# quzefan/LuSh-NeRF

Measured on AMD Instinct MI355X. Metric: training rays/sec (fwd+bwd), N_samples=64+64, higher is better.
Workload: dtype f16 MFMA forward (one fp16 plane per operand, fp32 accumulate; render outputs within 3e-5 of the fp32 reference); backward fp16 MFMA (one plane, per-launch power-of-two loss scale), fp32 accumulate; 1 GPU; poster_lushnerf 1xMI355X N_rand=4096/GPU N_samples=64 N_importance=64 blur kernel (DSK/RBK) on, fwd+bwd+Adam, one RCCL all-reduce of the flat gradient (BASELINE config C2); rays_per_gpu=4096, marched_rays_per_gpu=20480, planes_fwd=fp16x1, parallelism=dp1

## Files before the change

lush_nerf_amd/csrc/lush_mlp_dev.h:

```cpp
#pragma once
#include "lush_common.h"
#include "lush_mlp.h"

namespace lush {

__device__ __forceinline__ void lds_barrier() { asm volatile("s_waitcnt lgkmcnt(0)\n\ts_barrier" ::: "memory"); }

__device__ __forceinline__ unsigned mask_relayout(unsigned own, unsigned other, int h) {
    const unsigned w0 = h ? other : own, w1 = h ? own : other;
    const int sh = 4 * h;
    return ((w0 >> sh) & 0xFu) | (((w1 >> sh) & 0xFu) << 4) | (((w0 >> (8 + sh)) & 0xFu) << 8) | (((w1 >> (8 + sh)) & 0xFu) << 12);
}
__device__ __forceinline__ long long mask_index(int tile, int n_ml, int ml, int nrb, int rb, int CB, int cb) {
    return ((((long long)tile * CB + cb) * n_ml + ml) * nrb + rb) * 16;
}

template <int NS, int DT>
__device__ __forceinline__ void pe_put(char* img, int plane_bytes, int row_bytes, int pt, int col, float v) {
    __bf16 p[NS];
    split_planes<NS, DT>(v, p);
#pragma unroll
    for (int s = 0; s < NS; ++s)
        *reinterpret_cast<__bf16*>(img + s * plane_bytes + swz(pt, col >> 3, row_bytes) + (col & 7) * 2) = p[s];
}

__device__ __forceinline__ void point_of(const float* __restrict__ rays, const float* __restrict__ z,
                                         int S, long long gpt, float (&x)[3], float (&d)[3]) {
    const long long ray = gpt / S;
    const float zz = z[gpt];
    const float* rr = rays + ray * 11;
#pragma unroll
    for (int i = 0; i < 3; ++i) {
        x[i] = __fadd_rn(rr[i], __fmul_rn(rr[3 + i], zz));
        d[i] = rr[8 + i];
    }
}

__device__ __forceinline__ void lush_sincos(float x, float* sn, float* cs) {
    const float j = __builtin_rintf(__fmul_rn(x, 0.6366197723675814f));
    float r = __fmaf_rn(-j, 1.5707963705062866f, x);
    r = __fmaf_rn(-j, -4.371139000186243e-08f, r);
    r = __fmaf_rn(-j, -1.7151245100059906e-15f, r);
    const float z = __fmul_rn(r, r);
    float ps = __fmaf_rn(z, 0.0000027183114939898219064f, -0.000198393348360966317347f);
    ps = __fmaf_rn(z, ps, 0.0083333293858894631756f);
    ps = __fmaf_rn(z, ps, -0.166666666416265235595f);
    const float s = __fmaf_rn(__fmul_rn(z, r), ps, r);
    float pc = __fmaf_rn(z, 0.0000243904487962774090654f, -0.00138867637746099294692f);
    pc = __fmaf_rn(z, pc, 0.0416666233237390631894f);
    pc = __fmaf_rn(z, pc, -0.499999997251031003120f);
    const float c = __fmaf_rn(z, pc, 1.0f);
    const int q = (int)j;
    const float a = (q & 1) ? c : s, b = (q & 1) ? s : c;
    *sn = (q & 2) ? -a : a;
    *cs = ((q + 1) & 2) ? -b : b;
}

__device__ __forceinline__ void rev_split(float x, float* hi, float* lo) {
    constexpr float C_HI = 0.15915494309189535f;
    constexpr float C_LO = (float)(0.15915494309189533576888 - (double)C_HI);
    *hi = x * C_HI;
    *lo = __builtin_fmaf(x, C_HI, -*hi) + x * C_LO;
}
__device__ __forceinline__ void sincos_rev(float hi, float lo, int k, float* sn, float* cs) {
    const float s = (float)(1 << k);
    const float r = __builtin_amdgcn_fractf(hi * s) + lo * s;
    *sn = __builtin_amdgcn_sinf(r);
    *cs = __builtin_amdgcn_cosf(r);
}

template <int NS, int MT, int NTHREADS, int DT>
__device__ __noinline__ void pe_tile(char* peimg, int plane_bytes, int row_bytes, const float* rays, const float* z,
                                        int S, int P, long long tile_pt0, int tid, const int* live = nullptr) {
    constexpr int PARTS = NTHREADS / MT;
    const int pt = tid % MT, part = tid / MT;
    const long long gpt = tile_pt0 + pt;
    float x[3] = {0.f, 0.f, 0.f}, d[3] = {0.f, 0.f, 0.f};
    if (gpt < P) point_of(rays, z, S, live ? (long long)live[gpt] : gpt, x, d);
    for (int u = part; u < L_X + L_D; u += PARTS) {
        const bool isd = u >= L_X;
        const int k = isd ? u - L_X : u;
        const int base = isd ? PE_X : 0;
        const float f = (float)(1 << k);
#pragma unroll
        for (int i = 0; i < 3; ++i) {
            const float v = isd ? d[i] : x[i];
            if (k == 0) pe_put<NS, DT>(peimg, plane_bytes, row_bytes, pt, base + i, v);
            float s, c;
            lush_sincos(v * f, &s, &c);
            pe_put<NS, DT>(peimg, plane_bytes, row_bytes, pt, base + 3 + 6 * k + i, s);
            pe_put<NS, DT>(peimg, plane_bytes, row_bytes, pt, base + 3 + 6 * k + 3 + i, c);
        }
    }
    if (part == PARTS - 1) {
        pe_put<NS, DT>(peimg, plane_bytes, row_bytes, pt, PE_X_VALID, 0.f);
#pragma unroll
        for (int c = PE_X + PE_D_VALID; c < PE_X + PE_D; ++c) pe_put<NS, DT>(peimg, plane_bytes, row_bytes, pt, c, 0.f);
    }
}

__device__ __forceinline__ void dma16(const void* gptr, unsigned lds_base ) {
    unsigned keep;
    asm volatile("s_mov_b32 %0, m0\n\ts_mov_b32 m0, %2\n\ts_nop 0\n\tglobal_load_lds_dwordx4 %1, off\n\ts_mov_b32 m0, %0"
                 : "=&s"(keep) : "v"(gptr), "s"(lds_base) : "memory");
}

__device__ __forceinline__ void dma16s(const void* sbase , unsigned voff, unsigned lds_base ) {
    unsigned keep;
    asm volatile("s_mov_b32 %0, m0\n\ts_mov_b32 m0, %3\n\ts_nop 0\n\tglobal_load_lds_dwordx4 %1, %2\n\ts_mov_b32 m0, %0"
                 : "=&s"(keep) : "v"(voff), "s"(sbase), "s"(lds_base) : "memory");
}

__device__ __forceinline__ void dma16s_stream(const void* sbase , unsigned voff, unsigned lds_base ) {
    unsigned keep;
    asm volatile("s_mov_b32 %0, m0\n\ts_mov_b32 m0, %3\n\ts_nop 0\n\tglobal_load_lds_dwordx4 %1, %2 nt\n\ts_mov_b32 m0, %0"
                 : "=&s"(keep) : "v"(voff), "s"(sbase), "s"(lds_base) : "memory");
}

__device__ __forceinline__ void dma16s_x2(const void* sbase, unsigned voff0, unsigned lds0, unsigned voff1, unsigned lds1) {
    unsigned keep;
    asm volatile("s_mov_b32 %0, m0\n\ts_mov_b32 m0, %3\n\ts_nop 0\n\tglobal_load_lds_dwordx4 %1, %2\n\t"
                 "s_mov_b32 m0, %5\n\ts_nop 0\n\tglobal_load_lds_dwordx4 %4, %2\n\ts_mov_b32 m0, %0"
                 : "=&s"(keep) : "v"(voff0), "s"(sbase), "s"(lds0), "v"(voff1), "s"(lds1) : "memory");
}

}
```

lush_nerf_amd/csrc/lush_mlp_wide.hip:

```cpp
#include "lush_mlp_wide.h"
#include "lush_host.h"

#include <cstdio>
#include <cstdlib>
#include <utility>

namespace lush {

constexpr int WD_PE_PITCH = PE_ROW * 2 + 16;
constexpr int WD_PE_PLANE = WD_MT * WD_PE_PITCH;
constexpr int WD_PE_LIVE = (PE_X + PE_D) * 2;
static_assert(WD_PE_LIVE + 4 <= WD_PE_PITCH, "a row has room for the point's grid index");
constexpr int WD_SB = 2;
enum { WB_NONE = 0, WB_REG = 1, WB_PEX = 2, WB_PED = 3 };
enum { WC_NONE = 0, WC_ACT = 1, WC_ALPHA = 2 };

constexpr int WD_WRAP = NetNerf::fwd4_len / 8;
static_assert(NetNerf::fwd4_len % 8 == 0, "the quarter-row stream is whole positions");
constexpr int WD_TR_JUMP = 4 + 7 * 16 + 4;
constexpr int WD_TR_ALPHA = WD_TR_JUMP + 16;
constexpr int WD_TR_WRAP = WD_TR_JUMP + 2;
static_assert(WD_TR_ALPHA + 2 + 10 + 1 == WD_WRAP && WD_TR_WRAP == 122, "trunk | feature | alpha | views | rgb");
static_assert(WD_S < WD_TR_JUMP, "the prologue's positions are plain trunk positions");

LUSH_CLOCK_DECL(lush_clock_wide_fwd)

struct WdRt {
    bool pre_on;
    unsigned clamp;
    char* mptr[2];
    unsigned lane2;
    const float* nextbias;
    char* tile;
    char* srows;
    unsigned soff[2];
    unsigned srow_off;
};

typedef __attribute__((ext_vector_type(2))) unsigned short u16x2;
struct WdConvTmp {
    unsigned o[4];
    unsigned m;
    unsigned word[4];
};

template <int NRQP, int KB0, bool MASK>
struct WdConv {
    static constexpr int NB = 2 * NRQP;
    static constexpr int UPT = MASK ? 8 : 4;
    static constexpr int UPB = 2 * UPT;
    static constexpr int NVU = NB * UPB;

    template <int K>
    static __device__ __forceinline__ void unit(f32x16 (&pend)[2][2], u32x4 (&xout)[2][16], WdConvTmp& t, unsigned clamp) {
        constexpr int b = K / UPB, r = K % UPB, tt = r / UPT, u = r % UPT;
        constexpr int c = b % 2, rbl = b / 2, kb = KB0 + 2 * rbl + tt;
        constexpr int kind = MASK ? ((u == 0 || u == 1 || u == 3 || u == 5) ? 0 : 1) : 0;
        constexpr int i = MASK ? (kind == 0 ? (u == 0 ? 0 : (u == 1 ? 1 : (u == 3 ? 2 : 3))) : (u == 2 ? 0 : (u == 4 ? 1 : (u == 6 ? 2 : 3)))) : u;
        if constexpr (kind == 0) {
            unsigned o;
            asm volatile("v_cvt_pk_f16_f32 %0, %1, %2\n\tv_pk_max_i16 %0, %0, %3"
                         : "=&v"(o) : "v"(pend[c][rbl][8 * tt + 2 * i]), "v"(pend[c][rbl][8 * tt + 2 * i + 1]), "s"(clamp));
            t.o[i] = o;
            if constexpr (i == 3) {
                const u32x4 v = {t.o[0], t.o[1], t.o[2], t.o[3]};
                xout[c][kb] = v;
            }
        } else {
            constexpr int sh = 8 * tt + 2 * i;
            unsigned z;
            if constexpr (tt == 0 && i == 0) {
                asm volatile("v_pk_sub_u16 %0, 1, %1 op_sel_hi:[0,1] clamp" : "=v"(t.m) : "v"(t.o[i]));
            } else if constexpr (tt == 1 && i == 3) {
                unsigned w;
                asm volatile("v_pk_sub_u16 %1, 1, %3 op_sel_hi:[0,1] clamp\n\tv_lshl_or_b32 %2, %1, %4, %2\n\tv_lshrrev_b32 %1, 15, %2\n\tv_or_b32 %1, %1, %2\n\tv_not_b32 %0, %1"
                             : "=v"(w), "=&v"(z), "+v"(t.m) : "v"(t.o[i]), "n"(sh));
                t.word[b] = w;
            } else {
                asm volatile("v_pk_sub_u16 %0, 1, %2 op_sel_hi:[0,1] clamp\n\tv_lshl_or_b32 %1, %0, %3, %1" : "=&v"(z), "+v"(t.m) : "v"(t.o[i]), "n"(sh));
            }
        }
    }
};


template <int NRQ, int NPOS, int BMAIN, int KB0, int PRE, int CK, int NRQP, int CKB0, bool MASK, int NRQN, int D, int PQ, bool STASH, int LD, bool TRUNK = false>
struct WdPass {
    static constexpr int KBPP = 8 / NRQ;
    static constexpr int NG = NPOS * 16;
    static constexpr int DG = D < NG ? D : NG;
    using CV = WdConv<NRQP, CKB0, MASK>;
    static constexpr int NBLK = CK == WC_ACT ? CV::NB : 0;
    static constexpr int IPB = CK == WC_ACT ? CV::UPB + 5 : 0;
    static constexpr int NIT = NBLK * IPB;
    static_assert(BMAIN == WB_REG || NPOS == 1, "a PE-image segment is one position");
    static_assert(!STASH || NPOS == 4, "the stash pipeline is laid out over the 16 positions of a layer");

    struct Regs {
        bf16x8 a1[4];
        u32x4 bpe[2][4];
        WdConvTmp ct;
        unsigned dma_dst, dma_off;
    };

    static constexpr int ST_JOBS = 8;
    static constexpr bool st_write(int g) { return STASH && g % 16 >= 12 && (4 * PQ + g / 16) < ST_JOBS; }
    static constexpr bool st_read(int g) { return STASH && g % 16 >= 12 && (4 * PQ + g / 16) >= 1 && (4 * PQ + g / 16) <= ST_JOBS; }
    static constexpr int st_store_job(int g) {
        const int P = 4 * PQ + g / 16, m = g % 16;
        const int J = m >= 14 ? P - 1 : (m < 2 ? P - 2 : -1);
        return (STASH && J >= 0 && J < ST_JOBS) ? J : -1;
    }
    static constexpr int st_store_row(int g) { return g % 16 >= 14 ? g % 16 - 14 : g % 16 + 2; }
    static constexpr bool st_store(int g) { return st_store_job(g) >= 0; }

    static constexpr int item_weight(int k) {
        const int r = k % (IPB > 0 ? IPB : 1), b = k / (IPB > 0 ? IPB : 1);
        if (r < CV::UPB) {
            if (!MASK) return 3;
            const int u = r % CV::UPT;
            return (u == 0 || u == 1 || u == 3 || u == 5) ? 3 : 2;
        }
        if (r == CV::UPB) return MASK ? 2 : 0;
        return (b / 2) < NRQN ? 1 : 0;
    }
    static constexpr int fixed_load(int g) {
        const int m = g % 16;
        int w = 0;
        if (m < 4) w += 1;
        if (m == 4 || m == 5) w += 3;
        if (m == 8) w += 10;
        if (m >= 9 && m <= 11) w += 1;
        if (st_write(g)) w += 1;
        if (st_read(g)) w += 1;
        if (st_store(g)) w += 2;
        return w;
    }
    struct Sched {
        int first[NG + 1];
        int cap;
    };
    static constexpr Sched make_sched() {
        Sched S{};
        for (int cap = 6; cap < 64; ++cap) {
            int k = 0;
            for (int g = 0; g < NG; ++g) {
                S.first[g] = k;
                int load = fixed_load(g);
                if (g < DG || g == NG - 1) {
                    while (k < NIT) {
                        const int w = item_weight(k);
                        if (w > 0 && load + w > cap && !(g == NG - 1)) break;
                        load += w;
                        ++k;
                    }
                }
            }
            S.first[NG] = k;
            S.cap = cap;
            int last = 0;
            for (int g = 0; g < NG; ++g)
                if (S.first[g + 1] > S.first[g]) last = g;
            if (k == NIT && (last < DG || NIT == 0)) return S;
        }
        return S;
    }
    static constexpr Sched SC = make_sched();

    template <int SRC, int NKB>
    static __device__ __forceinline__ void load_bpe(Regs& r, const char* peimg, int row0, int lane) {
        const int n = lane & 31, hh = lane >> 5;
        const char* p = peimg + (row0 + n) * WD_PE_PITCH + hh * 16;
#pragma unroll
        for (int c = 0; c < 2; ++c)
#pragma unroll
            for (int k = 0; k < NKB; ++k)
                r.bpe[c][k] = *reinterpret_cast<const u32x4*>(p + c * 32 * WD_PE_PITCH + ((SRC == WB_PED ? PE_X / 8 : 0) + 2 * k) * 16);
    }

    template <int SRC, int NRQ_, int I, int M>
    static __device__ __forceinline__ void mfma(f32x16 (&act)[2][2], const Regs& r, const WdCarry& cr, const u32x4 (&xin)[2][16]) {
        constexpr int u = M / 2, c = M % 2;
        constexpr int kbl = NRQ_ == 2 ? u / 2 : u, rbl = NRQ_ == 2 ? u % 2 : 0;
        const bf16x8 a = u < 4 ? cr.a0[u] : r.a1[u - 4];
        if constexpr (SRC == WB_REG) act[c][rbl] = mfma_f16(a, __builtin_bit_cast(bf16x8, xin[c][KB0 + I * (8 / NRQ_) + kbl]), act[c][rbl]);
        else act[c][rbl] = mfma_f16(a, __builtin_bit_cast(bf16x8, r.bpe[c][SRC == WB_PED ? kbl % 2 : kbl]), act[c][rbl]);
    }

    template <int M>
    static __device__ __forceinline__ void fixed(WdCtx& cx, Regs& r, WdCarry& cr, const char* rd, const char* rd_next) {
        if constexpr (M < 4) {
            r.a1[M] = *reinterpret_cast<const bf16x8*>(rd + (4 + M) * 1024 + cx.lane * 16);
        } else if constexpr (M == 4) {
            r.dma_dst = cx.dma_base + cx.slot_off;
            r.dma_off = cx.fetch_off;
        } else if constexpr (M == 5) {
            if constexpr (TRUNK) {
                const unsigned f = cx.fetch_off + WD_SLOT == (unsigned)WD_TR_JUMP * WD_SLOT ? (unsigned)WD_TR_ALPHA * WD_SLOT : cx.fetch_off + WD_SLOT;
                cx.fetch_off = f == (unsigned)(WD_TR_ALPHA + 2) * WD_SLOT ? 0u : f;
            } else {
                cx.fetch_off = cx.fetch_off + WD_SLOT == (unsigned)WD_WRAP * WD_SLOT ? 0u : cx.fetch_off + WD_SLOT;
            }
            cx.slot_off = cx.slot_off + WD_SLOT == (unsigned)WD_S * WD_SLOT ? 0u : cx.slot_off + WD_SLOT;
        } else if constexpr (M == 8) {
            wd_dma_pair(cx.gbase + r.dma_off, cx.gbase + r.dma_off + 4096u, cx.voff, r.dma_dst, r.dma_dst + 4096u);
            cr.a0[0] = *reinterpret_cast<const bf16x8*>(rd_next + cx.lane * 16);
        } else if constexpr (M >= 9 && M <= 11) {
            cr.a0[M - 8] = *reinterpret_cast<const bf16x8*>(rd_next + (M - 8) * 1024 + cx.lane * 16);
        }
    }

    template <int K>
    static __device__ __forceinline__ void item(f32x16 (&pend)[2][2], u32x4 (&xout)[2][16], Regs& r, const WdRt& rt, int lane) {
        constexpr int b = K / IPB, rr = K % IPB, c = b % 2, rbl = b / 2;
        if constexpr (rr < CV::UPB) {
            CV::template unit<b * CV::UPB + rr>(pend, xout, r.ct, rt.clamp);
        } else if constexpr (rr == CV::UPB) {
            if constexpr (MASK) *reinterpret_cast<unsigned short*>(rt.mptr[c] + rbl * 128 + rt.lane2) = (unsigned short)r.ct.word[b];
        } else if constexpr (rbl < NRQN) {
            constexpr int j = rr - CV::UPB;
            const f32x4 v = *reinterpret_cast<const f32x4*>(rt.nextbias + rbl * 32 + 8 * (lane >> 5) + (j == 1 ? 0 : j == 2 ? 4 : j == 3 ? 16 : 20));
#pragma unroll
            for (int e = 0; e < 4; ++e) pend[c][rbl][4 * (j - 1) + e] = v[e];
        }
    }

    template <int G>
    static __device__ __forceinline__ void pending(f32x16 (&pend)[2][2], u32x4 (&xout)[2][16], Regs& r, const WdRt& rt, int lane, float (&alpha)[2]) {
        if constexpr (CK == WC_ACT) {
            wd_unroll<SC.first[G], SC.first[G + 1]>([&](auto kc) __attribute__((always_inline)) { item<decltype(kc)::value>(pend, xout, r, rt, lane); });
        } else if constexpr (CK == WC_ALPHA) {
            if constexpr (G == 0) {
                alpha[0] = pend[0][0][0];
                alpha[1] = pend[1][0][0];
            }
            if constexpr (G == 1) {
                asm volatile("" ::"v"(pend[0][0]), "v"(pend[1][0]));
            }
            if constexpr (G >= 1 && G <= 8) {
                constexpr int q = G - 1, c = q % 2, rbl = (q / 2) % 2, jj = q / 4;
                if constexpr (rbl < NRQN) {
#pragma unroll
                    for (int j2 = 0; j2 < 2; ++j2) {
                        const int j = 1 + 2 * jj + j2;
                        const f32x4 v = *reinterpret_cast<const f32x4*>(rt.nextbias + rbl * 32 + 8 * (lane >> 5) + (j == 1 ? 0 : j == 2 ? 4 : j == 3 ? 16 : 20));
#pragma unroll
                        for (int e = 0; e < 4; ++e) pend[c][rbl][4 * (j - 1) + e] = v[e];
                    }
                }
            }
        }
    }

    template <int JOB, int I4>
    static __device__ __forceinline__ void stash_store(const WdCarry& cr, const WdRt& rt) {
        constexpr int c = JOB / 4, j = JOB % 4;
        __builtin_nontemporal_store(cr.sb[I4 % WD_SB], reinterpret_cast<u32x4*>(rt.srows + ((c * 32 + 8 * I4) * LD + j * 64) * 2 + rt.srow_off));
    }
    template <int G>
    static __device__ __forceinline__ void stash(const u32x4 (&xin)[2][16], WdCarry& cr, const WdRt& rt, int lane) {
        constexpr int P = 4 * PQ + G / 16, m = G % 16;
        if constexpr (st_store(G)) stash_store<st_store_job(G), st_store_row(G)>(cr, rt);
        if constexpr (st_write(G)) {
            constexpr int job = P, c = job / 4, j = job % 4, o = m - 12;
            const int n = lane & 31, hh = lane >> 5;
            *reinterpret_cast<u32x4*>(rt.tile + (job % 2) * 4096 + n * 128 + (((2 * o + hh) ^ (n & 7)) << 4)) = xin[c][4 * j + o];
        }
        if constexpr (st_read(G)) {
            constexpr int job = P - 1, i = m - 12;
            const int row = 8 * i + (lane >> 3);
            cr.sb[i % WD_SB] = *reinterpret_cast<const u32x4*>(rt.tile + (job % 2) * 4096 + row * 128 + (((lane & 7) ^ (row & 7)) << 4));
        }
    }

    static constexpr int stores_in(int g0, int g1) {
        int n = 0;
        for (int g = g0 < 0 ? 0 : g0; g < g1 && g < NG; ++g) {
            if (st_store(g)) ++n;
            if (CK == WC_ACT && MASK)
                for (int k = SC.first[g]; k < SC.first[g + 1]; ++k)
                    if (k % IPB == CV::UPB) ++n;
        }
        return n;
    }

    template <int SRC, int NRQ_, int I, bool MAIN>
    static __device__ __forceinline__ void position(WdCtx& cx, f32x16 (&act)[2][2], f32x16 (&pend)[2][2], const u32x4 (&xin)[2][16],
                                                    u32x4 (&xout)[2][16], Regs& r, WdCarry& cr, const char* peimg, int row0, const WdRt& rt,
                                                    float (&alpha)[2]) {
        if constexpr (SRC != WB_REG) load_bpe<SRC, (SRC == WB_PED ? 2 : 4)>(r, peimg, row0, cx.lane);
        const char* rd = cx.ring + cx.slot_off;
        __builtin_amdgcn_sched_barrier(0);
        wd_unroll<0, 8>([&](auto mc) __attribute__((always_inline)) {
            constexpr int M = decltype(mc)::value;
            mfma<SRC, NRQ_, I, M>(act, r, cr, xin);
            fixed<M>(cx, r, cr, rd, nullptr);
            if constexpr (MAIN) {
                stash<16 * I + M>(xin, cr, rt, cx.lane);
                pending<16 * I + M>(pend, xout, r, rt, cx.lane, alpha);
            }
            __builtin_amdgcn_sched_barrier(0);
        });
        constexpr int younger = 2 * (WD_S - 2) + (MAIN ? stores_in(16 * (I + 1 - WD_S) + 8, 16 * I + 8) : 0);
        wd_wait_vm<(younger < 63 ? younger : 63)>();
        lds_barrier();
        const char* rd_next = cx.ring + cx.slot_off;
        __builtin_amdgcn_sched_barrier(0);
        wd_unroll<8, 16>([&](auto mc) __attribute__((always_inline)) {
            constexpr int M = decltype(mc)::value;
            mfma<SRC, NRQ_, I, M>(act, r, cr, xin);
            fixed<M>(cx, r, cr, rd, rd_next);
            if constexpr (MAIN) {
                stash<16 * I + M>(xin, cr, rt, cx.lane);
                pending<16 * I + M>(pend, xout, r, rt, cx.lane, alpha);
            }
            __builtin_amdgcn_sched_barrier(0);
        });
    }

    static __device__ __forceinline__ void run(WdCtx& cx, f32x16 (&act)[2][2], f32x16 (&pend)[2][2], const u32x4 (&xin)[2][16],
                                               u32x4 (&xout)[2][16], WdCarry& cr, const char* peimg, int row0, const WdRt& rt, float (&alpha)[2]) {
        Regs r;
        if constexpr (PRE == WB_PEX) {
            if (rt.pre_on) position<WB_PEX, 2, 0, false>(cx, act, pend, xin, xout, r, cr, peimg, row0, rt, alpha);
        } else if constexpr (PRE == WB_PED) {
            position<WB_PED, 2, 0, false>(cx, act, pend, xin, xout, r, cr, peimg, row0, rt, alpha);
        }
        wd_unroll<0, NPOS>([&](auto ic) __attribute__((always_inline)) {
            position<BMAIN, NRQ, decltype(ic)::value, true>(cx, act, pend, xin, xout, r, cr, peimg, row0, rt, alpha);
        });

    }
};

__device__ __noinline__ void wd_pe_tile(char* peimg, const float* rays, const float* z, int S, int P, long long tile_pt0, int tid, float* xd,
                                        const int* live) {
    const long long gpt = tile_pt0 + tid;
    float x[3] = {0.f, 0.f, 0.f}, d[3] = {0.f, 0.f, 0.f};
    if (gpt < P) point_of(rays, z, S, live ? (long long)live[gpt] : gpt, x, d);
    if (xd != nullptr) {
        float4* o = reinterpret_cast<float4*>(xd + gpt * 8);
        o[0] = make_float4(x[0], x[1], x[2], 0.f);
        o[1] = make_float4(d[0], d[1], d[2], 0.f);
    }
    float v[PE_X + PE_D];
#pragma unroll
    for (int c = 0; c < PE_X + PE_D; ++c) v[c] = 0.f;
#pragma unroll
    for (int i = 0; i < 3; ++i) {
        v[i] = x[i];
        v[PE_X + i] = d[i];
        float hx, lx, hd, ld;
        rev_split(x[i], &hx, &lx);
        rev_split(d[i], &hd, &ld);
#pragma unroll
        for (int k = 0; k < L_X; ++k) sincos_rev(hx, lx, k, &v[3 + 6 * k + i], &v[3 + 6 * k + 3 + i]);
#pragma unroll
        for (int k = 0; k < L_D; ++k) sincos_rev(hd, ld, k, &v[PE_X + 3 + 6 * k + i], &v[PE_X + 3 + 6 * k + 3 + i]);
    }
    char* row = peimg + tid * WD_PE_PITCH;
    if (live) *reinterpret_cast<int*>(row + WD_PE_LIVE) = gpt < P ? live[gpt] : 0;
#pragma unroll
    for (int c = 0; c < (PE_X + PE_D) / 8; ++c) {
        u32x4 w;
#pragma unroll
        for (int j = 0; j < 4; ++j) {
            unsigned o[1];
            split_pair<1, DT_F16>(v[8 * c + 2 * j], v[8 * c + 2 * j + 1], o);
            w[j] = o[0];
        }
        *reinterpret_cast<u32x4*>(row + c * 16) = w;
    }
}

__device__ __forceinline__ void wd_bias(f32x16 (&acc)[2][2], const float* b, int h, int nrq) {
#pragma unroll
    for (int c = 0; c < 2; ++c)
#pragma unroll
        for (int rbl = 0; rbl < 2; ++rbl) {
            if (rbl < nrq) {
                const f32x4* p = reinterpret_cast<const f32x4*>(b + rbl * 32 + 8 * h);
                const f32x4 v0 = p[0], v1 = p[1], v2 = p[4], v3 = p[5];
#pragma unroll
                for (int e = 0; e < 4; ++e) {
                    acc[c][rbl][e] = v0[e];
                    acc[c][rbl][4 + e] = v1[e];
                    acc[c][rbl][8 + e] = v2[e];
                    acc[c][rbl][12 + e] = v3[e];
                }
            }
        }
}

template <class N, int SPK, bool TRUNK = false>
__global__ __launch_bounds__(WD_NT) void mlp_wide_fwd_kernel(const MlpFwdArgs A) {
    static_assert(N::HW == 256 && N::NL == 8 && N::HV == 128, "the wide kernel is built for the 8x256 net");
    static_assert(!TRUNK || SPK == 0, "the trunk-only pass over all points keeps no stash");
    static_assert(!TRUNK || N::SKIP < N::NL - 1,"layer 7 of the trunk-only pass is a plain layer");
    constexpr int HW = N::HW, HV = N::HV, NL = N::NL, NRB = N::NRB;
    constexpr int NBIAS = N::f32_w_rgb;
    constexpr bool MASK = SPK > 0;
    constexpr int ML_BYTES = NRB * 128;
    constexpr int CB_BYTES = N::n_mask_layers * ML_BYTES;
    LUSH_CLOCK_STAMP(lush_clock_wide_fwd, 0);
    extern __shared__ __attribute__((aligned(16))) char smem[];
    float* biasl = reinterpret_cast<float*>(smem);
    char* ring = smem + NBIAS * 4;
    char* stage = ring + WD_S * WD_SLOT;
    char* peimg = stage + 8 * 4096;

    const int tid = threadIdx.x, lane = tid & 63;
    const int w = __builtin_amdgcn_readfirstlane(tid >> 6);
    const int n = lane & 31, h = lane >> 5;
    const char* wbase = reinterpret_cast<const char*>(A.wpk);
    {
        const float* f32 = reinterpret_cast<const float*>(wbase + (long long)N::total_entries * 1024);
        for (int i = tid; i < NBIAS; i += WD_NT) biasl[i] = f32[i];
    }
    WdCtx cx;
    cx.ring = ring;
    cx.ring_lds = (unsigned)(size_t)(__attribute__((address_space(3))) char*)ring;
    cx.gbase = wbase + (long long)N::fwd4_base * 1024;
    cx.slot_off = 0;
    cx.fetch_off = (unsigned)(WD_S % WD_WRAP) * WD_SLOT;
    cx.dma_base = __builtin_amdgcn_readfirstlane(cx.ring_lds + (unsigned)w * 1024u);
    cx.w = w;
    cx.lane = lane;
    cx.voff = (unsigned)lane * 16u + (unsigned)w * 1024u;
#pragma unroll
    for (int j = 0; j < WD_S; ++j)
        wd_dma_pair(cx.gbase + (unsigned)j * WD_SLOT, cx.gbase + (unsigned)j * WD_SLOT + 4096u, cx.voff, cx.dma_base + (unsigned)j * WD_SLOT, cx.dma_base + (unsigned)j * WD_SLOT + 4096u);

    const int row0 = w * 64;
    WdRt rt;
    rt.tile = stage + w * 8192;
    rt.pre_on = false;
    rt.srows = nullptr;
#pragma unroll
    for (int c = 0; c < 2; ++c) rt.soff[c] = (unsigned)(((c * 32 + n) * HW + h * 8) * 2);
    rt.srow_off = (unsigned)(((lane >> 3) * HW + (lane & 7) * 8) * 2);
    rt.lane2 = (unsigned)lane * 2u;
    float alpha[2] = {0.f, 0.f};
    int P = A.P, n_tiles = A.n_tiles;
    if (A.live_cnt != nullptr) {
        P = __builtin_amdgcn_readfirstlane(*A.live_cnt);
        n_tiles = (P + WD_MT - 1) / WD_MT;
    }

    for (int tile = blockIdx.x; tile < n_tiles; tile += gridDim.x) {
        const long long pt0 = (long long)tile * WD_MT;
        const long long wpt = pt0 + row0;
        wd_pe_tile(peimg, A.rays, A.z, A.S, P, pt0, tid, (SPK > 0 && !A.pe_rows) ? A.xd : nullptr, A.live_idx);
        if (tile == (int)blockIdx.x) wd_wait_vm<2 * (WD_S - 1)>();
        else wd_wait_vm<2 * (WD_S - 1) + (SPK > 0 ? 17 : 1)>();
        lds_barrier();
        if (SPK > 0 && A.pe_rows) {
            for (int i = tid; i < WD_MT * 12; i += WD_NT) {
                const int c = i % 12, pt = i / 12;
                const uint4 v = *reinterpret_cast<const uint4*>(peimg + pt * WD_PE_PITCH + c * 16);
                *reinterpret_cast<uint4*>(A.pe + (pt0 + pt) * PE_ROW + c * 8) = v;
            }
        }
        {
            unsigned long long gb = (unsigned long long)cx.gbase;
            asm volatile("" : "+s"(gb));
            cx.gbase = (const char*)gb;
        }
        char* mbase[2];
#pragma unroll
        for (int c = 0; c < 2; ++c) mbase[c] = reinterpret_cast<char*>(A.mask) + (wpt / 32 + c) * CB_BYTES;
        char* mdummy = reinterpret_cast<char*>(A.mask_dummy);
        auto mset = [&](int ml, int rb, bool dummy) __attribute__((always_inline)) {
#pragma unroll
            for (int c = 0; c < 2; ++c) rt.mptr[c] = dummy ? mdummy + c * 256 : mbase[c] + ml * ML_BYTES + rb * 128;
        };

        f32x16 accA[2][2], accB[2][2];
        u32x4 B0[2][16], B1[2][16];
        WdCarry a0;
#pragma unroll
        for (int i = 0; i < 4; ++i) a0.a0[i] = *reinterpret_cast<const bf16x8*>(cx.ring + cx.slot_off + i * 1024 + lane * 16);
        const float* btr = biasl + N::f32_b_trunk;
        wd_bias(accA, btr, h, 2);
        wd_bias(accB, btr + 64, h, 2);

        rt.clamp = 0u;
        WdPass<2, 1, WB_PEX, 0, WB_NONE, WC_NONE, 2, 0, MASK, 2, 16, 0, false, HW, TRUNK>::run(cx, accA, accB, B0, B0, a0, peimg, row0, rt, alpha);
        mset(0, 0, false); rt.nextbias = btr + 128;
        WdPass<2, 1, WB_PEX, 0, WB_NONE, WC_ACT, 2, 0, MASK, 2, 16, 0, false, HW, TRUNK>::run(cx, accB, accA, B0, B0, a0, peimg, row0, rt, alpha);
        mset(0, 2, false); rt.nextbias = btr + 192;
        WdPass<2, 1, WB_PEX, 0, WB_NONE, WC_ACT, 2, 4, MASK, 2, 16, 0, false, HW, TRUNK>::run(cx, accA, accB, B0, B0, a0, peimg, row0, rt, alpha);
        mset(0, 4, false); rt.nextbias = btr + HW;
        WdPass<2, 1, WB_PEX, 0, WB_NONE, WC_ACT, 2, 8, MASK, 2, 16, 0, false, HW, TRUNK>::run(cx, accB, accA, B0, B0, a0, peimg, row0, rt, alpha);

        auto layer = [&](int l, u32x4 (&xin)[2][16], u32x4 (&xout)[2][16]) __attribute__((always_inline)) {
            const bool feat = l == NL;
            const float* bl = btr + l * HW;
            rt.pre_on = l == N::SKIP;
            rt.srows = reinterpret_cast<char*>(A.h0 + (long long)(l - 1) * A.h_stride + wpt * HW);
            rt.clamp = 0u; mset(l - 1, 6, false); rt.nextbias = bl + 64;
            WdPass<2, 4, WB_REG, 0, WB_PEX, WC_ACT, 2, 12, MASK, 2, 48, 0, (SPK > 0), HW, TRUNK>::run(cx, accA, accB, xin, xin, a0, peimg, row0, rt, alpha);
            rt.clamp = feat ? 0x80008000u : 0u;
            mset(l, 0, feat); rt.nextbias = bl + 128;
            WdPass<2, 4, WB_REG, 0, WB_PEX, WC_ACT, 2, 0, MASK, 2, 60, 1, (SPK > 0), HW, TRUNK>::run(cx, accB, accA, xin, xout, a0, peimg, row0, rt, alpha);
            mset(l, 2, feat); rt.nextbias = bl + 192;
            WdPass<2, 4, WB_REG, 0, WB_PEX, WC_ACT, 2, 4, MASK, 2, 60, 2, (SPK > 0), HW, TRUNK>::run(cx, accA, accB, xin, xout, a0, peimg, row0, rt, alpha);
            mset(l, 4, feat); rt.nextbias = (feat || (TRUNK && l == NL - 1)) ? biasl + N::f32_b_alpha : bl + HW;
            WdPass<2, 4, WB_REG, 0, WB_PEX, WC_ACT, 2, 8, MASK, 2, 60, 3, (SPK > 0), HW, TRUNK>::run(cx, accB, accA, xin, xout, a0, peimg, row0, rt, alpha);
        };
#pragma unroll 1
        for (int l2 = 0; l2 < (TRUNK ? NL / 2 - 1 : NL / 2); ++l2) {
            layer(1 + 2 * l2, B0, B1);
            layer(2 + 2 * l2, B1, B0);
        }
        if constexpr (TRUNK) {
            layer(NL - 1, B0, B1);
            {
                WdConvTmp ct;
                using CV = WdConv<2, 12, false>;
                wd_unroll<0, CV::NVU>([&](auto kc) __attribute__((always_inline)) { CV::template unit<decltype(kc)::value>(accB, B1, ct, 0u); });
            }
            rt.pre_on = false;
            WdPass<1, 2, WB_REG, 0, WB_NONE, WC_NONE, 2, 0, false, 2, 16, 0, false, HW, TRUNK>::run(cx, accA, accB, B1, B1, a0, peimg, row0, rt, alpha);
            if (h == 0) {
#pragma unroll
                for (int c = 0; c < 2; ++c) {
                    const long long gpt = wpt + c * 32 + n;
                    if (gpt < P) *reinterpret_cast<float4*>(A.raw + gpt * 4) = make_float4(0.f, 0.f, 0.f, accA[c][0][0]);
                }
            }
            continue;
        }
        rt.pre_on = false;
        rt.clamp = 0x80008000u; mset(0, 0, true); rt.nextbias = biasl + N::f32_b_views;
        WdPass<1, 2, WB_REG, 0, WB_NONE, WC_ACT, 2, 12, MASK, 2, 32, 0, false, HW, TRUNK>::run(cx, accA, accB, B1, B0, a0, peimg, row0, rt, alpha);
        rt.nextbias = biasl + N::f32_b_views + 64;
        WdPass<2, 4, WB_REG, 0, WB_PED, WC_ALPHA, 1, 0, MASK, 2, 60, 0, false, HW, TRUNK>::run(cx, accB, accA, B0, B0, a0, peimg, row0, rt, alpha);
        rt.clamp = 0u; mset(NL, 0, false); rt.nextbias = biasl + N::f32_b_rgb;
        WdPass<2, 4, WB_REG, 0, WB_PED, WC_ACT, 2, 0, MASK, 1, 60, 0, false, HW, TRUNK>::run(cx, accA, accB, B0, B1, a0, peimg, row0, rt, alpha);
        {
            WdConvTmp ct;
            using CV = WdConv<2, 4, MASK>;
            mset(NL, 2, false);
            wd_unroll<0, CV::NVU>([&](auto kc) __attribute__((always_inline)) { CV::template unit<decltype(kc)::value>(accA, B1, ct, 0u); });
            if constexpr (MASK) {
#pragma unroll
                for (int b = 0; b < 4; ++b) *reinterpret_cast<unsigned short*>(rt.mptr[b % 2] + (b / 2) * 128 + rt.lane2) = (unsigned short)ct.word[b];
            }
        }
        if constexpr (SPK > 0) {
            char* hvrows = reinterpret_cast<char*>(A.hv + wpt * HV);
#pragma unroll
            for (int c = 0; c < 2; ++c)
#pragma unroll
                for (int j = 0; j < N::KKV / 4; ++j) {
#pragma unroll
                    for (int kq = 0; kq < 4; ++kq)
                        *reinterpret_cast<u32x4*>(rt.tile + n * 128 + (((2 * kq + h) ^ (n & 7)) << 4)) = B1[c][4 * j + kq];
#pragma unroll
                    for (int i = 0; i < 4; ++i) {
                        const int row = 8 * i + (lane >> 3);
                        const u32x4 v = *reinterpret_cast<const u32x4*>(rt.tile + row * 128 + (((lane & 7) ^ (row & 7)) << 4));
                        __builtin_nontemporal_store(v, reinterpret_cast<u32x4*>(hvrows + ((c * 32 + 8 * i) * HV + j * 64) * 2 + (unsigned)(((lane >> 3) * HV + (lane & 7) * 8) * 2)));
                    }
                }
        }
        WdPass<1, 1, WB_REG, 0, WB_NONE, WC_NONE, 2, 0, MASK, 2, 16, 0, false, HW, TRUNK>::run(cx, accB, accA, B1, B1, a0, peimg, row0, rt, alpha);
        if (h == 0) {
#pragma unroll
            for (int c = 0; c < 2; ++c) {
                const long long gpt = wpt + c * 32 + n;
                if (gpt < P && A.raw != nullptr) {
                    float4 o;
                    o.x = accB[c][0][0];
                    o.y = accB[c][0][1];
                    o.z = accB[c][0][2];
                    o.w = alpha[c];
                    const long long dst = A.live_idx != nullptr ? (long long)*reinterpret_cast<const int*>(peimg + (row0 + c * 32 + n) * WD_PE_PITCH + WD_PE_LIVE) : gpt;
                    *reinterpret_cast<float4*>(A.raw + dst * 4) = o;
                }
            }
        }
    }
    wd_wait_vm<0>();
    LUSH_CLOCK_STAMP(lush_clock_wide_fwd, 1);
}

LUSH_CLOCK_EXPORT(lush_debug_clock_fwd, lush_clock_wide_fwd)
static_assert((NetNerf::f32_w_rgb * 4) % 16 == 0, "the ring behind the bias block stays 16-byte aligned");
size_t mlp_wide_fwd_lds_bytes() { return (size_t)WD_S * WD_SLOT + (size_t)WD_PE_PLANE + (size_t)NetNerf::f32_w_rgb * 4 + 8 * 4096; }

template <int SPK, bool TRUNK = false>
static int launch_wide_sp(const MlpFwdArgs& a, hipStream_t s) {
    auto k = mlp_wide_fwd_kernel<NetNerf, SPK, TRUNK>;
    const size_t lds = mlp_wide_fwd_lds_bytes();
    static KernelOnce once;
    int dev = 0, n_cu = 0;
    if (int rc = current_device_cus(dev, n_cu)) return rc;
    if (int rc = kernel_lds_once(once, dev, reinterpret_cast<const void*>(k), lds)) return rc;
    const int tiles = (a.n_tiles * 128 + WD_MT - 1) / WD_MT;
    MlpFwdArgs b = a;
    b.n_tiles = tiles;
    const int grid = tiles < n_cu ? tiles : n_cu;
    hipLaunchKernelGGL(k, dim3(grid), dim3(WD_NT), lds, s, b);
    LUSH_HIP(hipGetLastError());
    return 0;
}

int launch_mlp_wide_fwd(const MlpFwdArgs& a, hipStream_t s) {
    const int sp = a.write_stash ? a.stash_planes : 0;
    if (a.trunk_only) {
        if (sp != 0 || a.live_idx || !a.raw) return set_error("launch_mlp_wide_fwd: the trunk-only pass runs over all the points, without stash");
        return launch_wide_sp<0, true>(a, s);
    }
    if (sp == 0) return launch_wide_sp<0>(a, s);
    if (sp == 1) return launch_wide_sp<1>(a, s);
    return set_error("launch_mlp_wide_fwd: one stash plane at most");
}

}
```

Before: 372,400 rays/s.

## Interleave next tile's positional encoding into last trunk layer MFMA gaps

In the trunk-only forward pass, the per-tile positional encoding of the next tile is split into small units (load, combine, range-reduce, sin, cos, pack, store) and scheduled into the idle slots between MFMA steps of the last trunk layer. A compile-time plan caps the extra per-step load. The point data for the next tile is prefetched with direct-to-LDS dword DMAs, and only the first tile runs the standalone encoding (xyz only). This aims to hide the encoding's ALU and latency cost behind matrix work, at the cost of more register pressure, tighter wait counts and more complex scheduling. Optional clock stamps per tile are added under a debug flag.

```diff
diff --git a/lush_nerf_amd/csrc/lush_mlp_dev.h b/lush_nerf_amd/csrc/lush_mlp_dev.h
--- a/lush_nerf_amd/csrc/lush_mlp_dev.h
+++ b/lush_nerf_amd/csrc/lush_mlp_dev.h
@@ -62,9 +62,12 @@
     *hi = x * C_HI;
     *lo = __builtin_fmaf(x, C_HI, -*hi) + x * C_LO;
 }
+__device__ __forceinline__ float sincos_rev_arg(float hi, float lo, int k) {
+    const float s = (float)(1 << k);
+    return __builtin_amdgcn_fractf(hi * s) + lo * s;
+}
 __device__ __forceinline__ void sincos_rev(float hi, float lo, int k, float* sn, float* cs) {
-    const float s = (float)(1 << k);
-    const float r = __builtin_amdgcn_fractf(hi * s) + lo * s;
+    const float r = sincos_rev_arg(hi, lo, k);
     *sn = __builtin_amdgcn_sinf(r);
     *cs = __builtin_amdgcn_cosf(r);
 }
@@ -111,6 +114,12 @@
                  : "=&s"(keep) : "v"(voff), "s"(sbase), "s"(lds_base) : "memory");
 }
 
+__device__ __forceinline__ void dma4s(const void* sbase , unsigned voff, unsigned lds_base ) {
+    unsigned keep;
+    asm volatile("s_nop 4\n\ts_mov_b32 %0, m0\n\ts_mov_b32 m0, %3\n\ts_nop 0\n\tglobal_load_lds_dword %1, %2\n\ts_mov_b32 m0, %0"
+                 : "=&s"(keep) : "v"(voff), "s"(sbase), "s"(lds_base) : "memory");
+}
+
 __device__ __forceinline__ void dma16s_stream(const void* sbase , unsigned voff, unsigned lds_base ) {
     unsigned keep;
     asm volatile("s_mov_b32 %0, m0\n\ts_mov_b32 m0, %3\n\ts_nop 0\n\tglobal_load_lds_dwordx4 %1, %2 nt\n\ts_mov_b32 m0, %0"
diff --git a/lush_nerf_amd/csrc/lush_mlp_wide.hip b/lush_nerf_amd/csrc/lush_mlp_wide.hip
--- a/lush_nerf_amd/csrc/lush_mlp_wide.hip
+++ b/lush_nerf_amd/csrc/lush_mlp_wide.hip
@@ -24,6 +24,16 @@
 static_assert(WD_S < WD_TR_JUMP, "the prologue's positions are plain trunk positions");
 
 LUSH_CLOCK_DECL(lush_clock_wide_fwd)
+#ifdef LUSH_CLOCK
+constexpr int WD_TS_WG = 256, WD_TS_TILES = 48;
+__device__ unsigned long long lush_clock_trunk_tiles[WD_TS_WG][WD_TS_TILES][4];
+#define WD_TILE_STAMP(on, lt, k, expr)                                                                       \
+    do {                                                                                                     \
+        if ((on) && threadIdx.x == 0 && blockIdx.x < WD_TS_WG && (lt) < WD_TS_TILES) lush_clock_trunk_tiles[blockIdx.x][lt][k] = (expr); \
+    } while (0)
+#else
+#define WD_TILE_STAMP(on, lt, k, expr)
+#endif
 
 struct WdRt {
     bool pre_on;
@@ -83,8 +93,141 @@
     }
 };
 
-
-template <int NRQ, int NPOS, int BMAIN, int KB0, int PRE, int CK, int NRQP, int CKB0, bool MASK, int NRQN, int D, int PQ, bool STASH, int LD, bool TRUNK = false>
+constexpr int WD_ENC_DMAS = 7;
+static_assert(WD_S - 1 >= 4, "the point DMAs are younger than the ring DMA of every mid-step of layer 0");
+#ifndef LUSH_ENC_CAP
+#define LUSH_ENC_CAP 7
+#endif
+#ifndef LUSH_ENC_LAG
+#define LUSH_ENC_LAG 1
+#endif
+constexpr int WD_ENC_CAP = LUSH_ENC_CAP;
+constexpr int WD_ENC_LAG = LUSH_ENC_LAG;
+#define WD_PIN(x) asm volatile("" : "+v"(x))
+typedef __attribute__((address_space(3))) const float* wd_lds_cf;
+typedef __attribute__((address_space(3))) u32x4* wd_lds_q;
+
+struct WdEncIn {
+    const float* rays;
+    const float* z;
+    int S, P;
+    long long wpt;
+    unsigned stg;
+    unsigned rows;
+};
+struct WdEnc {
+    float hi[3], lo[3];
+    float w[3];
+    float r;
+    float v[PE_X];
+    unsigned pk[PE_X / 2];
+    unsigned voff;
+    const char* sray;
+};
+
+struct WdEncUnits {
+    enum { XL = 0, XC = 1, RR = 2, SN = 3, CS = 4 };
+    static constexpr int NU = 6 + 9 * L_X;
+    static constexpr int kind(int n) { return n < 6 ? n % 2 : 2 + (n - 6) % 3; }
+    static constexpr int coord(int n) { return n < 6 ? n / 2 : ((n - 6) / 3) % 3; }
+    static constexpr int freq(int n) { return n < 6 ? 0 : (n - 6) / 9; }
+    static constexpr int col_unit(int c) {
+        if (c < 3) return 2 * c + 1;
+        const int k = (c - 3) / 6, r = (c - 3) % 6;
+        return 6 + 3 * (3 * k + r % 3) + (r < 3 ? 1 : 2);
+    }
+    static constexpr int pair_unit(int j) {
+        const int a = col_unit(2 * j), b = 2 * j + 1 == PE_X_VALID ? 0 : col_unit(2 * j + 1);
+        const int u = (a > b ? a : b) + WD_ENC_LAG;
+        return u < NU ? u : NU - 1;
+    }
+    static constexpr int chunk_unit(int c) {
+        int u = 0;
+        for (int j = 4 * c; j < 4 * c + 4; ++j) u = pair_unit(j) > u ? pair_unit(j) : u;
+        return u + WD_ENC_LAG < NU ? u + WD_ENC_LAG : NU - 1;
+    }
+    static constexpr int weight(int n) {
+        int w = kind(n) == XL ? 3 : (kind(n) == XC ? 6 : 4);
+        for (int j = 0; j < PE_X / 2; ++j) w += pair_unit(j) == n ? 1 : 0;
+        for (int c = 0; c < PE_X / 8; ++c) w += chunk_unit(c) == n ? 1 : 0;
+        return w;
+    }
+
+    static __device__ __forceinline__ void load0(WdEnc& e, const WdEncIn& in, int lane) {
+        const bool any = in.wpt < in.P;
+        const unsigned wv = any ? (unsigned)in.wpt : 0u;
+        const int nv = any ? (in.P - (int)wv < 64 ? in.P - (int)wv : 64) : 1;
+        const unsigned l = lane < nv ? (unsigned)lane : 0u;
+        const unsigned ray = (wv + l) / (unsigned)in.S;
+        const unsigned ray_w = __builtin_amdgcn_readfirstlane(ray);
+        e.voff = (ray - ray_w) * 44u;
+        e.sray = wd_uniform(reinterpret_cast<const char*>(in.rays + (long long)ray_w * 11));
+        dma4s(wd_uniform(reinterpret_cast<const char*>(in.z + wv)), l * 4u, in.stg);
+        WD_PIN(e.voff);
+    }
+    static __device__ __forceinline__ void load1(WdEnc& e, const WdEncIn& in) {
+        unsigned keep;
+        asm volatile("s_mov_b32 %0, m0\n\ts_mov_b32 m0, %3\n\ts_nop 0\n\tglobal_load_lds_dword %1, %2\n\t"
+                     "v_add_u32 %1, 4, %1\n\ts_add_u32 m0, m0, 0x100\n\ts_nop 0\n\tglobal_load_lds_dword %1, %2\n\t"
+                     "v_add_u32 %1, 4, %1\n\ts_add_u32 m0, m0, 0x100\n\ts_nop 0\n\tglobal_load_lds_dword %1, %2\n\t"
+                     "v_add_u32 %1, 4, %1\n\ts_add_u32 m0, m0, 0x100\n\ts_nop 0\n\tglobal_load_lds_dword %1, %2\n\t"
+                     "v_add_u32 %1, 4, %1\n\ts_add_u32 m0, m0, 0x100\n\ts_nop 0\n\tglobal_load_lds_dword %1, %2\n\t"
+                     "v_add_u32 %1, 4, %1\n\ts_add_u32 m0, m0, 0x100\n\ts_nop 0\n\tglobal_load_lds_dword %1, %2\n\t"
+                     "s_mov_b32 m0, %0"
+                     : "=&s"(keep), "+v"(e.voff) : "s"(e.sray), "s"(in.stg + 256u) : "memory", "scc");
+    }
+
+    template <int J>
+    static __device__ __forceinline__ void pack(WdEnc& e) {
+        unsigned o[1];
+        split_pair<1, DT_F16>(e.v[2 * J], 2 * J + 1 == PE_X_VALID ? 0.f : e.v[2 * J + 1], o);
+        e.pk[J] = o[0];
+        WD_PIN(e.pk[J]);
+    }
+    template <int K>
+    static __device__ __forceinline__ void unit(WdEnc& e, const WdEncIn& in, int lane) {
+        constexpr int kd = kind(K), i = coord(K), k = freq(K);
+        if constexpr (kd == XL) {
+            unsigned a = in.stg + (unsigned)lane * 4u;
+            WD_PIN(a);
+            e.w[0] = *(wd_lds_cf)(a);
+            e.w[1] = *(wd_lds_cf)(a + (1 + i) * 256u);
+            e.w[2] = *(wd_lds_cf)(a + (4 + i) * 256u);
+        } else if constexpr (kd == XC) {
+            WD_PIN(e.w[0]); WD_PIN(e.w[1]); WD_PIN(e.w[2]);
+            const float x = in.wpt + lane < in.P ? __fadd_rn(e.w[1], __fmul_rn(e.w[2], e.w[0])) : 0.f;
+            e.v[i] = x;
+            rev_split(x, &e.hi[i], &e.lo[i]);
+            WD_PIN(e.v[i]); WD_PIN(e.hi[i]); WD_PIN(e.lo[i]);
+        } else if constexpr (kd == RR) {
+            WD_PIN(e.hi[i]); WD_PIN(e.lo[i]);
+            e.r = sincos_rev_arg(e.hi[i], e.lo[i], k);
+            WD_PIN(e.r);
+        } else if constexpr (kd == SN) {
+            WD_PIN(e.r);
+            e.v[3 + 6 * k + i] = __builtin_amdgcn_sinf(e.r);
+            WD_PIN(e.v[3 + 6 * k + i]);
+        } else {
+            WD_PIN(e.r);
+            e.v[3 + 6 * k + 3 + i] = __builtin_amdgcn_cosf(e.r);
+            WD_PIN(e.v[3 + 6 * k + 3 + i]);
+        }
+        wd_unroll<0, PE_X / 2>([&](auto jc) __attribute__((always_inline)) {
+            if constexpr (pair_unit(decltype(jc)::value) == K) pack<decltype(jc)::value>(e);
+        });
+        wd_unroll<0, PE_X / 8>([&](auto cc) __attribute__((always_inline)) {
+            constexpr int c = decltype(cc)::value;
+            if constexpr (chunk_unit(c) == K) {
+                const u32x4 q = {e.pk[4 * c], e.pk[4 * c + 1], e.pk[4 * c + 2], e.pk[4 * c + 3]};
+                *(wd_lds_q)(in.rows + (unsigned)lane * WD_PE_PITCH + c * 16u) = q;
+            }
+        });
+    }
+};
+template <int LD> struct WdEncPlan;
+
+
+template <int NRQ, int NPOS, int BMAIN, int KB0, int PRE, int CK, int NRQP, int CKB0, bool MASK, int NRQN, int D, int PQ, bool STASH, int LD, bool TRUNK = false, int ENC = 0>
 struct WdPass {
     static constexpr int KBPP = 8 / NRQ;
     static constexpr int NG = NPOS * 16;
@@ -95,6 +238,7 @@
     static constexpr int NIT = NBLK * IPB;
     static_assert(BMAIN == WB_REG || NPOS == 1, "a PE-image segment is one position");
     static_assert(!STASH || NPOS == 4, "the stash pipeline is laid out over the 16 positions of a layer");
+    static_assert(ENC <= 0 || (TRUNK && NPOS == 4 && !STASH && !MASK && PQ == ENC - 1), "the encoding units fill the last trunk layer of the trunk-only pass");
 
     struct Regs {
         bf16x8 a1[4];
@@ -284,10 +428,16 @@
         return n;
     }
 
+    template <int G>
+    static __device__ __forceinline__ void enc_gap(WdEnc& e, const WdEncIn& in, int lane) {
+        using PL = WdEncPlan<LD>;
+        wd_unroll<PL::P.first[G], PL::P.first[G + 1]>([&](auto kc) __attribute__((always_inline)) { WdEncUnits::template unit<decltype(kc)::value>(e, in, lane); });
+    }
+
     template <int SRC, int NRQ_, int I, bool MAIN>
     static __device__ __forceinline__ void position(WdCtx& cx, f32x16 (&act)[2][2], f32x16 (&pend)[2][2], const u32x4 (&xin)[2][16],
                                                     u32x4 (&xout)[2][16], Regs& r, WdCarry& cr, const char* peimg, int row0, const WdRt& rt,
-                                                    float (&alpha)[2]) {
+                                                    float (&alpha)[2], WdEnc* en, const WdEncIn* ein) {
         if constexpr (SRC != WB_REG) load_bpe<SRC, (SRC == WB_PED ? 2 : 4)>(r, peimg, row0, cx.lane);
         const char* rd = cx.ring + cx.slot_off;
         __builtin_amdgcn_sched_barrier(0);
@@ -298,10 +448,11 @@
             if constexpr (MAIN) {
                 stash<16 * I + M>(xin, cr, rt, cx.lane);
                 pending<16 * I + M>(pend, xout, r, rt, cx.lane, alpha);
+                if constexpr (ENC > 0) enc_gap<64 * (ENC - 1) + 16 * I + M>(*en, *ein, cx.lane);
             }
             __builtin_amdgcn_sched_barrier(0);
         });
-        constexpr int younger = 2 * (WD_S - 2) + (MAIN ? stores_in(16 * (I + 1 - WD_S) + 8, 16 * I + 8) : 0);
+        constexpr int younger = 2 * (WD_S - 2) + (MAIN ? stores_in(16 * (I + 1 - WD_S) + 8, 16 * I + 8) : 0) + (ENC < 0 ? WD_ENC_DMAS : 0);
         wd_wait_vm<(younger < 63 ? younger : 63)>();
         lds_barrier();
         const char* rd_next = cx.ring + cx.slot_off;
@@ -313,26 +464,61 @@
             if constexpr (MAIN) {
                 stash<16 * I + M>(xin, cr, rt, cx.lane);
                 pending<16 * I + M>(pend, xout, r, rt, cx.lane, alpha);
+                if constexpr (ENC > 0) enc_gap<64 * (ENC - 1) + 16 * I + M>(*en, *ein, cx.lane);
             }
             __builtin_amdgcn_sched_barrier(0);
         });
     }
 
     static __device__ __forceinline__ void run(WdCtx& cx, f32x16 (&act)[2][2], f32x16 (&pend)[2][2], const u32x4 (&xin)[2][16],
-                                               u32x4 (&xout)[2][16], WdCarry& cr, const char* peimg, int row0, const WdRt& rt, float (&alpha)[2]) {
+                                               u32x4 (&xout)[2][16], WdCarry& cr, const char* peimg, int row0, const WdRt& rt, float (&alpha)[2],
+                                               WdEnc* en = nullptr, const WdEncIn* ein = nullptr) {
         Regs r;
         if constexpr (PRE == WB_PEX) {
-            if (rt.pre_on) position<WB_PEX, 2, 0, false>(cx, act, pend, xin, xout, r, cr, peimg, row0, rt, alpha);
+            if (rt.pre_on) position<WB_PEX, 2, 0, false>(cx, act, pend, xin, xout, r, cr, peimg, row0, rt, alpha, en, ein);
         } else if constexpr (PRE == WB_PED) {
-            position<WB_PED, 2, 0, false>(cx, act, pend, xin, xout, r, cr, peimg, row0, rt, alpha);
+            position<WB_PED, 2, 0, false>(cx, act, pend, xin, xout, r, cr, peimg, row0, rt, alpha, en, ein);
         }
         wd_unroll<0, NPOS>([&](auto ic) __attribute__((always_inline)) {
-            position<BMAIN, NRQ, decltype(ic)::value, true>(cx, act, pend, xin, xout, r, cr, peimg, row0, rt, alpha);
+            position<BMAIN, NRQ, decltype(ic)::value, true>(cx, act, pend, xin, xout, r, cr, peimg, row0, rt, alpha, en, ein);
         });
 
     }
 };
 
+template <int LD>
+struct WdEncPlan {
+    template <int Q>
+    using Twin = WdPass<2, 4, WB_REG, 0, WB_PEX, WC_ACT, 2, (Q == 0 ? 12 : 4 * (Q - 1)), false, 2, (Q == 0 ? 48 : 60), Q, false, LD, true, 0>;
+    struct Plan {
+        int first[4 * 64 + 1];
+    };
+    template <int Q>
+    static constexpr void pour(Plan& p, int& n) {
+        using T = Twin<Q>;
+        for (int g = 0; g < 64; ++g) {
+            const int G = 64 * Q + g;
+            p.first[G] = n;
+            int load = T::fixed_load(g);
+            for (int k = T::SC.first[g]; k < T::SC.first[g + 1]; ++k) load += T::item_weight(k);
+            if (n < WdEncUnits::NU && load + WdEncUnits::weight(n) <= WD_ENC_CAP) ++n;
+        }
+    }
+    static constexpr Plan make() {
+        Plan p{};
+        int n = 0;
+        pour<0>(p, n);
+        pour<1>(p, n);
+        pour<2>(p, n);
+        pour<3>(p, n);
+        p.first[4 * 64] = n;
+        return p;
+    }
+    static constexpr Plan P = make();
+    static_assert(P.first[4 * 64] == WdEncUnits::NU, "the layer's gaps take the whole encoding of a row");
+};
+
+template <bool GD = true>
 __device__ __noinline__ void wd_pe_tile(char* peimg, const float* rays, const float* z, int S, int P, long long tile_pt0, int tid, float* xd,
                                         const int* live) {
     const long long gpt = tile_pt0 + tid;
@@ -356,12 +542,12 @@
 #pragma unroll
         for (int k = 0; k < L_X; ++k) sincos_rev(hx, lx, k, &v[3 + 6 * k + i], &v[3 + 6 * k + 3 + i]);
 #pragma unroll
-        for (int k = 0; k < L_D; ++k) sincos_rev(hd, ld, k, &v[PE_X + 3 + 6 * k + i], &v[PE_X + 3 + 6 * k + 3 + i]);
+        for (int k = 0; k < (GD ? L_D : 0); ++k) sincos_rev(hd, ld, k, &v[PE_X + 3 + 6 * k + i], &v[PE_X + 3 + 6 * k + 3 + i]);
     }
     char* row = peimg + tid * WD_PE_PITCH;
     if (live) *reinterpret_cast<int*>(row + WD_PE_LIVE) = gpt < P ? live[gpt] : 0;
 #pragma unroll
-    for (int c = 0; c < (PE_X + PE_D) / 8; ++c) {
+    for (int c = 0; c < (GD ? PE_X + PE_D : PE_X) / 8; ++c) {
         u32x4 w;
 #pragma unroll
         for (int j = 0; j < 4; ++j) {
@@ -447,13 +633,34 @@
         n_tiles = (P + WD_MT - 1) / WD_MT;
     }
 
+    WdEncIn ein;
+    if constexpr (TRUNK) {
+        ein.rays = A.rays;
+        ein.z = A.z;
+        ein.S = A.S;
+        ein.P = P;
+        ein.stg = __builtin_amdgcn_readfirstlane((unsigned)(size_t)(__attribute__((address_space(3))) char*)rt.tile);
+        ein.rows = __builtin_amdgcn_readfirstlane((unsigned)(size_t)(__attribute__((address_space(3))) char*)(peimg + row0 * WD_PE_PITCH));
+    }
+    [[maybe_unused]] int lt = 0;
+
     for (int tile = blockIdx.x; tile < n_tiles; tile += gridDim.x) {
         const long long pt0 = (long long)tile * WD_MT;
         const long long wpt = pt0 + row0;
-        wd_pe_tile(peimg, A.rays, A.z, A.S, P, pt0, tid, (SPK > 0 && !A.pe_rows) ? A.xd : nullptr, A.live_idx);
-        if (tile == (int)blockIdx.x) wd_wait_vm<2 * (WD_S - 1)>();
-        else wd_wait_vm<2 * (WD_S - 1) + (SPK > 0 ? 17 : 1)>();
+        WD_TILE_STAMP(TRUNK, lt, 0, __builtin_amdgcn_s_memtime());
+        WD_TILE_STAMP(TRUNK, lt, 3, (unsigned long long)(tile != (int)blockIdx.x));
+        if constexpr (!TRUNK) wd_pe_tile(peimg, A.rays, A.z, A.S, P, pt0, tid, (SPK > 0 && !A.pe_rows) ? A.xd : nullptr, A.live_idx);
+        else if (tile == (int)blockIdx.x) wd_pe_tile<false>(peimg, A.rays, A.z, A.S, P, pt0, tid, nullptr, nullptr);
+        WdEnc en;
+        if constexpr (TRUNK) {
+            ein.wpt = (long long)(tile + (int)gridDim.x) * WD_MT + row0;
+            WdEncUnits::load0(en, ein, lane);
+            WdEncUnits::load1(en, ein);
+        }
+        if (tile == (int)blockIdx.x) wd_wait_vm<2 * (WD_S - 1) + (TRUNK ? WD_ENC_DMAS : 0)>();
+        else wd_wait_vm<2 * (WD_S - 1) + (SPK > 0 ? 17 : 1) + (TRUNK ? WD_ENC_DMAS : 0)>();
         lds_barrier();
+        WD_TILE_STAMP(TRUNK, lt, 1, __builtin_amdgcn_s_memtime());
         if (SPK > 0 && A.pe_rows) {
             for (int i = tid; i < WD_MT * 12; i += WD_NT) {
                 const int c = i % 12, pt = i / 12;
@@ -485,36 +692,37 @@
         wd_bias(accB, btr + 64, h, 2);
 
         rt.clamp = 0u;
-        WdPass<2, 1, WB_PEX, 0, WB_NONE, WC_NONE, 2, 0, MASK, 2, 16, 0, false, HW, TRUNK>::run(cx, accA, accB, B0, B0, a0, peimg, row0, rt, alpha);
+        WdPass<2, 1, WB_PEX, 0, WB_NONE, WC_NONE, 2, 0, MASK, 2, 16, 0, false, HW, TRUNK, (TRUNK ? -1 : 0)>::run(cx, accA, accB, B0, B0, a0, peimg, row0, rt, alpha);
         mset(0, 0, false); rt.nextbias = btr + 128;
-        WdPass<2, 1, WB_PEX, 0, WB_NONE, WC_ACT, 2, 0, MASK, 2, 16, 0, false, HW, TRUNK>::run(cx, accB, accA, B0, B0, a0, peimg, row0, rt, alpha);
+        WdPass<2, 1, WB_PEX, 0, WB_NONE, WC_ACT, 2, 0, MASK, 2, 16, 0, false, HW, TRUNK, (TRUNK ? -1 : 0)>::run(cx, accB, accA, B0, B0, a0, peimg, row0, rt, alpha);
         mset(0, 2, false); rt.nextbias = btr + 192;
-        WdPass<2, 1, WB_PEX, 0, WB_NONE, WC_ACT, 2, 4, MASK, 2, 16, 0, false, HW, TRUNK>::run(cx, accA, accB, B0, B0, a0, peimg, row0, rt, alpha);
+        WdPass<2, 1, WB_PEX, 0, WB_NONE, WC_ACT, 2, 4, MASK, 2, 16, 0, false, HW, TRUNK, (TRUNK ? -1 : 0)>::run(cx, accA, accB, B0, B0, a0, peimg, row0, rt, alpha);
         mset(0, 4, false); rt.nextbias = btr + HW;
-        WdPass<2, 1, WB_PEX, 0, WB_NONE, WC_ACT, 2, 8, MASK, 2, 16, 0, false, HW, TRUNK>::run(cx, accB, accA, B0, B0, a0, peimg, row0, rt, alpha);
-
-        auto layer = [&](int l, u32x4 (&xin)[2][16], u32x4 (&xout)[2][16]) __attribute__((always_inline)) {
+        WdPass<2, 1, WB_PEX, 0, WB_NONE, WC_ACT, 2, 8, MASK, 2, 16, 0, false, HW, TRUNK, (TRUNK ? -1 : 0)>::run(cx, accB, accA, B0, B0, a0, peimg, row0, rt, alpha);
+
+        auto layer = [&](int l, u32x4 (&xin)[2][16], u32x4 (&xout)[2][16], auto enc) __attribute__((always_inline)) {
+            constexpr int E = decltype(enc)::value;
             const bool feat = l == NL;
             const float* bl = btr + l * HW;
             rt.pre_on = l == N::SKIP;
             rt.srows = reinterpret_cast<char*>(A.h0 + (long long)(l - 1) * A.h_stride + wpt * HW);
             rt.clamp = 0u; mset(l - 1, 6, false); rt.nextbias = bl + 64;
-            WdPass<2, 4, WB_REG, 0, WB_PEX, WC_ACT, 2, 12, MASK, 2, 48, 0, (SPK > 0), HW, TRUNK>::run(cx, accA, accB, xin, xin, a0, peimg, row0, rt, alpha);
+            WdPass<2, 4, WB_REG, 0, WB_PEX, WC_ACT, 2, 12, MASK, 2, 48, 0, (SPK > 0), HW, TRUNK, E * 1>::run(cx, accA, accB, xin, xin, a0, peimg, row0, rt, alpha, &en, &ein);
             rt.clamp = feat ? 0x80008000u : 0u;
             mset(l, 0, feat); rt.nextbias = bl + 128;
-            WdPass<2, 4, WB_REG, 0, WB_PEX, WC_ACT, 2, 0, MASK, 2, 60, 1, (SPK > 0), HW, TRUNK>::run(cx, accB, accA, xin, xout, a0, peimg, row0, rt, alpha);
+            WdPass<2, 4, WB_REG, 0, WB_PEX, WC_ACT, 2, 0, MASK, 2, 60, 1, (SPK > 0), HW, TRUNK, E * 2>::run(cx, accB, accA, xin, xout, a0, peimg, row0, rt, alpha, &en, &ein);
             mset(l, 2, feat); rt.nextbias = bl + 192;
-            WdPass<2, 4, WB_REG, 0, WB_PEX, WC_ACT, 2, 4, MASK, 2, 60, 2, (SPK > 0), HW, TRUNK>::run(cx, accA, accB, xin, xout, a0, peimg, row0, rt, alpha);
+            WdPass<2, 4, WB_REG, 0, WB_PEX, WC_ACT, 2, 4, MASK, 2, 60, 2, (SPK > 0), HW, TRUNK, E * 3>::run(cx, accA, accB, xin, xout, a0, peimg, row0, rt, alpha, &en, &ein);
             mset(l, 4, feat); rt.nextbias = (feat || (TRUNK && l == NL - 1)) ? biasl + N::f32_b_alpha : bl + HW;
-            WdPass<2, 4, WB_REG, 0, WB_PEX, WC_ACT, 2, 8, MASK, 2, 60, 3, (SPK > 0), HW, TRUNK>::run(cx, accB, accA, xin, xout, a0, peimg, row0, rt, alpha);
+            WdPass<2, 4, WB_REG, 0, WB_PEX, WC_ACT, 2, 8, MASK, 2, 60, 3, (SPK > 0), HW, TRUNK, E * 4>::run(cx, accB, accA, xin, xout, a0, peimg, row0, rt, alpha, &en, &ein);
         };
 #pragma unroll 1
         for (int l2 = 0; l2 < (TRUNK ? NL / 2 - 1 : NL / 2); ++l2) {
-            layer(1 + 2 * l2, B0, B1);
-            layer(2 + 2 * l2, B1, B0);
+            layer(1 + 2 * l2, B0, B1, std::integral_constant<int, 0>{});
+            layer(2 + 2 * l2, B1, B0, std::integral_constant<int, 0>{});
         }
         if constexpr (TRUNK) {
-            layer(NL - 1, B0, B1);
+            layer(NL - 1, B0, B1, std::integral_constant<int, 1>{});
             {
                 WdConvTmp ct;
                 using CV = WdConv<2, 12, false>;
@@ -529,6 +737,8 @@
                     if (gpt < P) *reinterpret_cast<float4*>(A.raw + gpt * 4) = make_float4(0.f, 0.f, 0.f, accA[c][0][0]);
                 }
             }
+            WD_TILE_STAMP(TRUNK, lt, 2, __builtin_amdgcn_s_memtime());
+            ++lt;
             continue;
         }
         rt.pre_on = false;
@@ -587,6 +797,15 @@
 }
 
 LUSH_CLOCK_EXPORT(lush_debug_clock_fwd, lush_clock_wide_fwd)
+#ifdef LUSH_CLOCK
+extern "C" int lush_debug_clock_trunk_tiles(unsigned long long* out ) {
+    if (hipDeviceSynchronize() != hipSuccess) return -1;
+    if (hipMemcpyFromSymbol(out, HIP_SYMBOL(lush_clock_trunk_tiles), sizeof(lush_clock_trunk_tiles)) != hipSuccess) return -1;
+    void* p = nullptr;
+    if (hipGetSymbolAddress(&p, HIP_SYMBOL(lush_clock_trunk_tiles)) != hipSuccess) return -1;
+    return hipMemset(p, 0, sizeof(lush_clock_trunk_tiles)) == hipSuccess ? 0 : -1;
+}
+#endif
 static_assert((NetNerf::f32_w_rgb * 4) % 16 == 0, "the ring behind the bias block stays 16-byte aligned");
 size_t mlp_wide_fwd_lds_bytes() { return (size_t)WD_S * WD_SLOT + (size_t)WD_PE_PLANE + (size_t)NetNerf::f32_w_rgb * 4 + 8 * 4096; }
 
```

Result: no change. 373,900 rays/s, median of 6 (+0.4%).
